# kmkolasinski/tfrecords-reader

Hardware: AMD Instinct MI355X
Metric: GiB/s + examples/s device-resident TFRecord->Feature decode, 1/2/4/8 GPU (higher is better)
Workload: dtype u8; 1 GPU; C4 directory (configs[4]) of 256 files, C1-shaped (int64 label + 12 B bytes_list id) records, 524288 +-50 % per file (default_rng(1000+f)), spec CRC-32C; this rank's LPT share (256 files) resident in HBM; records_per_gpu=134295581, framed_bytes_per_gpu=7906235019, parallelism=file-sharded x1 (LPT by bytes, no collective on the data path), batches_per_gpu=4, batch_bytes_max=1976558779, streams=2, tpl_groups_missed=0

## Files before the change

### include/tfrg.h

```cpp
#ifndef TFRG_H
#define TFRG_H
#include <stdint.h>
#include "tfrg_status.h"

#ifdef __cplusplus
extern "C" {
#endif

#define TFRG_ABI_VERSION 1

#define TFRG_E_ARG (-1)
#define TFRG_E_HIP (-2)
#define TFRG_E_NOMEM (-3)
#define TFRG_E_IO (-4)
#define TFRG_E_LIMIT (-5)

#define TFRG_FLAG_PAYLOAD_ONLY 1u
#define TFRG_FLAG_SPEC_VARINT 2u
#define TFRG_FLAG_NO_CRC 4u
#define TFRG_FLAG_STRICT_CRC 8u
#define TFRG_FLAG_MATERIALIZE_BYTES 16u

int tfrg_abi_version(void);
const char* tfrg_status_exception(int status);
// ... 104 lines not shown
  uint32_t n_miss_entries;
  uint32_t n_big;
  uint32_t scan_timeout;
  uint64_t kind_totals[4];
  uint64_t nbytes;
  uint64_t bytes_data_len;
  uint32_t tpl_groups_missed;
  uint32_t implicit_cols;
  uint64_t placed_slots;
  uint64_t implicit_off_slots;
} tfrg_info;

int tfrg_ctx_rel_off(const tfrg_ctx* ctx, uint32_t slot, int32_t* delta);

int tfrg_result_info(tfrg_ctx* ctx, tfrg_info* info);

typedef struct tfrg_columns {
  int32_t* status;
  int64_t* aux;
  uint8_t* verdict;
  uint16_t* order;
  uint32_t* row_splits;
  uint64_t* slot_base;
  int64_t* i64;
  uint32_t* f32;
  uint32_t* bytes_off;
  uint32_t* bytes_len;
  uint32_t* miss;
  uint8_t* bytes_data;
  uint64_t* bytes_offsets;
} tfrg_columns;

int tfrg_result_device(tfrg_ctx* ctx, tfrg_columns* cols);
int tfrg_result_fetch(tfrg_ctx* ctx, const tfrg_columns* host);

#define TFRG_DENSE_I64 0
#define TFRG_DENSE_I32 1
#define TFRG_DENSE_F32 2
#define TFRG_DENSE_U8 3
#define TFRG_DENSE_MAX_SPECS 64
#define TFRG_DENSE_MAX_WIDTH 4096
typedef struct tfrg_dense_spec {
  uint32_t slot;
  uint32_t dtype;
  uint32_t width;
  uint32_t reserved;
  uint64_t fill;
  void* out;
  int32_t* lengths;
} tfrg_dense_spec;
int tfrg_result_dense(tfrg_ctx* ctx, const tfrg_dense_spec* specs, uint32_t n_specs, uint32_t* d_stats,
                      void* consumer_stream);

#define TFRG_ROWS_I32 0
#define TFRG_ROWS_I64 1
int tfrg_result_dense_rows(tfrg_ctx* ctx, const tfrg_dense_spec* specs, uint32_t n_specs, const void* d_rows,
                           uint32_t rows_dtype, uint32_t m, int64_t row0, uint32_t* d_stats, uint32_t* d_skipped,
                           void* consumer_stream);

#define TFRG_RAGGED_MAX_SPECS 64
typedef struct tfrg_ragged_spec {
  uint32_t slot;
  uint32_t dtype;
  uint32_t max_len;
  uint32_t reserved;
  uint64_t cap;
// ... 58 lines not shown
```

### tfrecords-reader_amd/csrc/tfrg_capi.cpp

```cpp
#include <hip/hip_runtime.h>
#include <stdlib.h>
#include <string.h>

#include <algorithm>
#include <map>
#include <numeric>
#include <string>
#include <unordered_map>
#include <vector>

#include "../../include/tfrg.h"
#include "crc32c.h"
#include "tfrg_dense.h"
#include "tfrg_ragged.h"
#include "tfrg_select.h"
#include "tfrg_frame.h"
#include "tfrg_internal.h"
#include "tfrg_learn.h"

namespace tfrg {
void set_error(const std::string& s);

#define HIP_TRY(expr)                                                              \
  do {                                                                             \
    hipError_t e_ = (expr);                                                        \
    if (e_ != hipSuccess) {                                                        \
      set_error(std::string(#expr) + ": " + hipGetErrorString(e_));               \
      return TFRG_E_HIP;                                                           \
    }                                                                              \
  } while (0)

struct DBuf {
  void* p = nullptr;
  size_t cap = 0;
  hipError_t ensure(size_t bytes) {
    if (bytes <= cap && p) return hipSuccess;
    if (p) {
      hipError_t e = hipFree(p);
      if (e != hipSuccess) return e;
      p = nullptr;
      cap = 0;
    }
    size_t want = bytes < 256 ? 256 : bytes;
    want = (want + 4095) & ~(size_t)4095;
    hipError_t e = hipMalloc(&p, want);
    if (e == hipSuccess) cap = want;
    return e;
  }
  void release() {
    if (p) (void)hipFree(p);
    p = nullptr;
// ... 70 lines not shown
  uint32_t tpl_frames = 0;
  bool tpl_on = true;
  std::vector<uint8_t> slot_kind_h;
  DBuf spec;
  std::vector<uint32_t> spec_h;
  bool have_spec = false;
  bool spec_on = true;
  bool profiling = false;
  bool have_events = false;
  hipEvent_t ev[kNumStages + 1] = {};
  uint64_t hint_i64 = 0, hint_f32 = 0, hint_b = 0;
  bool hinted = false;
  bool no_hints = false;
  uint64_t hint_reruns = 0;
  bool optimistic_on = true;
  bool walk_beside = true;
  uint32_t walk_blocks = 0;
  bool no_quiet = false;
  bool opt_pending = false;
  bool ord_const = false;
  bool len_const = false;
  std::vector<uint32_t> const_len;
  bool implicit_off_on = true;
  uint64_t off_rel = 0;
  std::vector<int32_t> rel_off;
  uint64_t last_off_mask = 0;
  std::vector<int32_t> last_rel_off;
  bool off_complete = false;
  uint32_t last_implicit = 0;
  bool last_aux_zero = false;
  uint32_t* info_pin = nullptr;
  bool cols_complete = false;
  bool mat_pending = false;
  struct LastCall {
    const uint8_t* d_bytes;
    uint64_t nbytes;
    uint64_t cap_in;
    uint64_t bound;
    uint32_t n, flags;
    hipStream_t st;
  } last{};
  Offsets last_off{};
  uint32_t index_chunk = kIndexChunkDefault;
  DBuf fr_tab, fr_dev;
  uint32_t ragged_tile = kRaggedTileDefault;
  DBuf rg_tsum;
  uint32_t select_tile = kSelTileDefault;
  DBuf sel_buf;
  void* fr_pin = nullptr;
  size_t fr_pin_cap = 0;
  uint32_t poison[4] = {0xffffffffu, 0xffffffffu, 0xffffffffu, 0xffffffffu};
};

extern "C" {

int tfrg_ctx_create(int device, tfrg_ctx** out) {
  *out = nullptr;
  int ndev = 0;
  HIP_TRY(hipGetDeviceCount(&ndev));
  if (device < 0 || device >= ndev) {
    set_error("bad device index");
    return TFRG_E_ARG;
  }
  HIP_TRY(hipSetDevice(device));
  tfrg_ctx* c = new tfrg_ctx();
  c->device = device;
  if (const char* e = getenv("TFRG_TEMPLATES")) c->tpl_on = atoi(e) != 0;
  if (const char* e = getenv("TFRG_SPEC")) c->spec_on = atoi(e) != 0;
  if (const char* e = getenv("TFRG_TPL_STAGE")) c->tpl_stage = atoi(e);
  if (const char* e = getenv("TFRG_TPL_GPW")) {
    const int v = atoi(e);
    if (v == 2 || v == 4 || v == 8) c->tpl_gpw = (uint32_t)v;
  }
  if (const char* e = getenv("TFRG_OPTIMISTIC")) c->optimistic_on = atoi(e) != 0;
  if (const char* e = getenv("TFRG_IMPLICIT_OFF")) c->implicit_off_on = atoi(e) != 0;
  if (const char* e = getenv("TFRG_WALK_BESIDE")) c->walk_beside = atoi(e) != 0;
  if (const char* e = getenv("TFRG_WALK_BLOCKS")) c->walk_blocks = (uint32_t)atoi(e);
  if (const char* e = getenv("TFRG_DENSE_NT")) c->dense_nt = atoi(e) != 0;
  if (const char* e = getenv("TFRG_DEBUG_POISON_LOC")) {
    char* q = const_cast<char*>(e);
    for (int i = 0; i < 4 && *q; ++i) {
      c->poison[i] = (uint32_t)strtoul(q, &q, 10);
      while (*q == ',' || *q == ' ') ++q;
    }
  }
  hipDeviceProp_t prop;
  if (hipGetDeviceProperties(&prop, device) == hipSuccess) {
    c->num_cus = prop.multiProcessorCount;
    if (prop.maxSharedMemoryPerMultiProcessor) c->cu_lds = (uint32_t)prop.maxSharedMemoryPerMultiProcessor;
  }
  if (hipStreamCreateWithFlags(&c->own_stream, hipStreamNonBlocking) != hipSuccess) {
    delete c;
    set_error("hipStreamCreate failed");
    return TFRG_E_HIP;
  }
  if (hipHostMalloc(reinterpret_cast<void**>(&c->info_pin), (kInfoCount + 8) * 4) != hipSuccess) {
    (void)hipStreamDestroy(c->own_stream);
    delete c;
    set_error("hipHostMalloc failed");
    return TFRG_E_NOMEM;
  }
  std::vector<uint32_t> tab(kCrcTabWords), cst(128);
  CrcTables T;
  crc_make_tables(&T);
  memcpy(tab.data(), T.t, 4096);
  uint32_t M[4][256];
  crc_make_mul_tables(gf_xpow8(1024), M);
  memcpy(tab.data() + 1024, M, 4096);
// ... 421 lines not shown
  uint32_t* const info = c->info.as<uint32_t>() + c->info_slot * kInfoCount;
  DevBytes d;
  d.in = d_bytes;
  d.in_readable = (nbytes + 15) & ~15ull;
  d.b_off = c->b_off.as<uint32_t>();
  d.b_len = c->b_len.as<uint32_t>();
  d.kind_totals = c->kind_totals.as<uint64_t>();
  d.offsets = c->boff64.as<uint64_t>();
  d.offsets_cap = cap_b;
  d.data = c->bdata.as<uint8_t>();
  d.data_cap = cap_in + 16;
  d.lb = c->blb.as<uint64_t>();
  d.ticket = info + kInfoBytesTicket;
  d.big_count = info + kInfoBytesBig;
  d.big_list = c->bbig.as<uint32_t>();
  d.overflow = info + kInfoOverflow;
  return launch_materialize(d, c->num_cus, st);
}

static int decode_device_any(tfrg_ctx* c, const uint8_t* d_bytes, uint64_t nbytes, const Offsets& off, uint32_t n,
                             uint32_t flags, void* stream) {
  if (!c) return TFRG_E_ARG;
  if (nbytes >= (1ull << 32)) {
    set_error("batch larger than 4 GiB: split it");
    return TFRG_E_LIMIT;
  }
  if (c->n_keys == 0) {
    uint64_t z = 0;
    int st = tfrg_set_schema(c, 0, nullptr, &z, nullptr, 0, nullptr, nullptr);
    if (st) return st;
  }
  HIP_TRY(hipSetDevice(c->device));
  c->have_result = false;
  hipStream_t st = stream ? (hipStream_t)stream : c->own_stream;
  if (flags & TFRG_FLAG_STRICT_CRC) flags &= ~TFRG_FLAG_NO_CRC;
  if (c->last_stream && c->last_stream != st) {
    if (!c->order_ev) HIP_TRY(hipEventCreateWithFlags(&c->order_ev, hipEventDisableTiming));
    HIP_TRY(hipEventRecord(c->order_ev, c->last_stream));
    HIP_TRY(hipStreamWaitEvent(st, c->order_ev, 0));
  }
  const uint32_t S = c->n_slots;
  const uint64_t nn = n ? n : 1;
  const uint64_t ngroups = (nn + 63) / 64;
  const uint32_t n_tiles = (n + kTileRecs - 1) / kTileRecs;
  const uint32_t tile_stride = (n_tiles + 3u) & ~3u;
  const uint32_t n_chunks = (n_tiles + (1u << kSpineChunkShift) - 1u) >> kSpineChunkShift;
  const uint64_t tsum_words = (uint64_t)S * tile_stride + 2ull * S * n_chunks + S;
  const uint64_t cap_in = c->cap_hint > nbytes ? c->cap_hint : nbytes;
  c->cap_hint = 0;
  uint64_t cap_i64 = cap_in + 16, cap_f32 = cap_in / 4 + 16, cap_b = cap_in / 2 + 16;
  c->hinted = false;
  auto hint = [&](uint64_t h, uint64_t& cap) {
    if (h && h + 16 < cap) {
      cap = h + 16;
      c->hinted = true;
    }
  };
  if (!c->no_hints) {
    hint(c->hint_i64, cap_i64);
    hint(c->hint_f32, cap_f32);
    hint(c->hint_b, cap_b);
  }
  bool grow = c->status.cap < nn * 4 || c->aux.cap < nn * 8 || c->verdict.cap < nn ||
              c->order.cap < S * nn * 2 || c->count.cap < S * nn * 4 || c->loc.cap < S * nn * 8 ||
              c->rs.cap < S * (nn + 1) * 4 || c->i64.cap < cap_i64 * 8 || c->f32.cap < cap_f32 * 4 ||
              c->b_off.cap < cap_b * 4 || c->b_len.cap < cap_b * 4 || c->big_list.cap < nn * 4 ||
              c->slow_list.cap < nn * 4 || c->tsum.cap < tsum_words * 4 + 16 || c->crc_rec.cap < nn * 4 ||
              c->crc_base.cap < nn * 8 || c->crc_part.cap < nn * 8 || c->lmask.cap < ngroups * 8 ||
              c->rlist.cap < ngroups * 4;
  if (grow && c->last_stream) HIP_TRY(hipStreamSynchronize(c->last_stream));
  const size_t tsum_cap0 = c->tsum.cap;
  if (c->status.ensure(nn * 4) || c->aux.ensure(nn * 8) || c->verdict.ensure(nn) || c->order.ensure(S * nn * 2) ||
      c->count.ensure(S * nn * 4) || c->loc.ensure(S * nn * 8) || c->rs.ensure(S * (nn + 1) * 4) ||
      c->slot_base.ensure((S + 1) * 8) || c->totals.ensure((S + 1) * 4) || c->kind_totals.ensure(32) ||
      c->i64.ensure(cap_i64 * 8) || c->f32.ensure(cap_f32 * 4) || c->b_off.ensure(cap_b * 4) ||
      c->b_len.ensure(cap_b * 4) || c->big_list.ensure(nn * 4) || c->slow_list.ensure(nn * 4) ||
      c->miss.ensure(kMissCap * 16ull) || c->info.ensure(2 * kInfoCount * 4) ||
      c->tsum.ensure(tsum_words * 4 + 16) || c->crc_rec.ensure(nn * 4) || c->crc_base.ensure(nn * 8) ||
      c->crc_part.ensure(nn * 8) || c->lmask.ensure(ngroups * 8) || c->rlist.ensure(ngroups * 4)) {
    set_error("device allocation failed");
    return TFRG_E_NOMEM;
  }
  const uint32_t islot = c->info_slot ^ 1u;
  uint32_t* const info_cur = c->info.as<uint32_t>() + islot * kInfoCount;
  if (!c->info_clean) HIP_TRY(hipMemsetAsync(info_cur, 0, kInfoCount * 4, st));
  c->info_clean = false;
  c->info_slot = islot;
  if (c->tsum.cap != tsum_cap0 || c->tsum_dirty) {
    HIP_TRY(hipMemsetAsync(c->tsum.p, 0, c->tsum.cap, st));
    HIP_TRY(hipMemsetAsync(c->status.p, 0, c->status.cap, st));
    c->tsum_dirty = false;
  }
  if (S && n == 0) HIP_TRY(hipMemsetAsync(c->rs.p, 0, S * 4, st));
  const bool mat = (flags & TFRG_FLAG_MATERIALIZE_BYTES) != 0;
  const uint64_t lb_words = materialize_lb_words(cap_b);
  if (mat) {
    const bool g2 = c->bdata.cap < cap_in + 16 || c->boff64.cap < (cap_b + 1) * 8 || c->blb.cap < lb_words * 8 ||
                    c->bbig.cap < cap_b * 4;
    if (g2 && c->last_stream) HIP_TRY(hipStreamSynchronize(c->last_stream));
    if (c->bdata.ensure(cap_in + 16) || c->boff64.ensure((cap_b + 1) * 8) || c->blb.ensure(lb_words * 8) ||
        c->bbig.ensure(cap_b * 4)) {
      set_error("device allocation failed (materialized bytes)");
      return TFRG_E_NOMEM;
    }
    HIP_TRY(hipMemsetAsync(c->blb.p, 0, lb_words * 8, st));
    if (!n) HIP_TRY(hipMemsetAsync(c->boff64.p, 0, 8, st));
  }
  if (!S || !n) HIP_TRY(hipMemsetAsync(c->kind_totals.p, 0, 32, st));

  DevBatch b;
  b.bytes = d_bytes;
  b.nbytes = nbytes;
  b.start = off.s64;
  b.end = off.e64;
  b.start32 = off.s32;
  b.end32 = off.e32;
  b.first = off.first;
  b.omode = off.mode;
  b.n = n;
  b.flags = flags;
  DevOut o;
// ... 91 lines not shown
    }
    hipError_t e = launch_decode(b, schema_view(c), o, cfg, c->crc_tab.as<uint32_t>(), c->consts.as<uint32_t>(), st, ev);
    if (e == hipSuccess && mat && S && !cfg.ran_optimistic) {
      e = launch_materialize_last(c, d_bytes, nbytes, cap_in, cap_b, st);
    } else if (e == hipSuccess && mat && !S) {
      e = hipMemsetAsync(c->boff64.p, 0, 8, st);
    }
    if (ev && e == hipSuccess) e = hipEventRecord(ev[kNumStages], st);
    if (e != hipSuccess) {
      c->tsum_dirty = true;
      set_error(std::string("kernel launch: ") + hipGetErrorString(e));
      return TFRG_E_HIP;
    }
  }
  c->info_clean = n != 0;
  c->n = n;
  c->nbytes = nbytes;
  c->cap_i64 = cap_i64;
  c->cap_f32 = cap_f32;
  c->cap_b = cap_b;
  c->last_stream = st;
  c->materialized = mat;
  c->have_result = true;
  c->rs_complete = false;
  c->opt_pending = n != 0 && cfg.ran_optimistic;
  if (n != 0 && cfg.ran_quiet_big) c->tsum_dirty = true;
  c->mat_pending = c->opt_pending && mat && S;
  c->last_implicit = n != 0 ? cfg.implicit : 0u;
  c->last_off_mask = n != 0 ? cfg.implicit_off : 0ull;
  if (c->last_off_mask) c->last_rel_off = c->rel_off;
  c->off_complete = false;
  c->last_aux_zero = n != 0 && cfg.ran_optimistic && !cfg.ran_quiet_big && !(cfg.implicit & TFRG_IMPLICIT_STATUS);
  c->cols_complete = false;
  return 0;
}

int tfrg_decode_host(tfrg_ctx* c, const uint8_t* h_bytes, uint64_t nbytes, const uint64_t* h_start,
                     const uint64_t* h_end, uint32_t n, uint32_t flags, void* stream) {
  if (!c) return TFRG_E_ARG;
  HIP_TRY(hipSetDevice(c->device));
  hipStream_t st = stream ? (hipStream_t)stream : c->own_stream;
  const uint64_t pad = ((nbytes + 15) & ~15ull) + 16;
  if (c->last_stream) HIP_TRY(hipStreamSynchronize(c->last_stream));
  if (c->in_bytes.ensure(pad) || c->in_start.ensure((uint64_t)(n ? n : 1) * 8) ||
      c->in_end.ensure((uint64_t)(n ? n : 1) * 8)) {
    set_error("staging allocation failed");
    return TFRG_E_NOMEM;
  }
  if (nbytes) HIP_TRY(hipMemcpyAsync(c->in_bytes.p, h_bytes, nbytes, hipMemcpyHostToDevice, st));
  HIP_TRY(hipMemsetAsync(c->in_bytes.as<uint8_t>() + nbytes, 0, pad - nbytes, st));
  if (n) {
    HIP_TRY(hipMemcpyAsync(c->in_start.p, h_start, (size_t)n * 8, hipMemcpyHostToDevice, st));
    HIP_TRY(hipMemcpyAsync(c->in_end.p, h_end, (size_t)n * 8, hipMemcpyHostToDevice, st));
  }
  uint64_t total = 0, widest = 0;
  for (uint32_t i = 0; i < n; ++i) {
    const uint64_t a = h_start[i], b = h_end[i] < nbytes ? h_end[i] : nbytes;
    if (b > a) total += b - a;
    if (h_end[i] > a && h_end[i] - a > widest) widest = h_end[i] - a;
  }
  if (!c->tpl_learned && c->n_keys && c->tpl_on) {
    const int t = tfrg_learn_templates(c, h_bytes, nbytes, h_start, h_end, n, flags);
    if (t < 0) return t;
  }
  c->cap_hint = total;
  c->call_bound = widest ? widest : 1;
  return tfrg_decode_device(c, c->in_bytes.as<uint8_t>(), nbytes, c->in_start.as<uint64_t>(),
                            c->in_end.as<uint64_t>(), n, flags, st);
}

static int finish_decode(tfrg_ctx* c, uint32_t* h, uint64_t* kt) {
  bool widened = false;
  for (;;) {
    HIP_TRY(hipMemcpyAsync(c->info_pin, c->info.as<uint32_t>() + c->info_slot * kInfoCount, kInfoCount * 4,
                           hipMemcpyDeviceToHost, c->last_stream));
    HIP_TRY(hipMemcpyAsync(c->info_pin + kInfoCount, c->kind_totals.p, 32, hipMemcpyDeviceToHost, c->last_stream));
    HIP_TRY(hipStreamSynchronize(c->last_stream));
    memcpy(h, c->info_pin, kInfoCount * 4);
    memcpy(kt, c->info_pin + kInfoCount, 32);
    const bool full = c->opt_pending && h[kInfoResid] != 0;
    const bool widen = h[kInfoOverflow] && c->hinted && !widened;
    if (!full && !widen) {
      if (!c->mat_pending) break;
      c->mat_pending = false;
      const tfrg_ctx::LastCall& L = c->last;
      HIP_TRY(launch_materialize_last(c, L.d_bytes, L.nbytes, L.cap_in, c->cap_b, c->last_stream));
      continue;
    }
    const tfrg_ctx::LastCall L = c->last;
    c->no_quiet = true;
    c->no_hints = widen;
    c->cap_hint = L.cap_in;
    c->call_bound = L.bound;
    c->tsum_dirty = true;
    const int rc = decode_device_any(c, L.d_bytes, L.nbytes, c->last_off, L.n, L.flags, L.st);
    c->no_quiet = false;
    c->no_hints = false;
    if (rc) return rc;
    widened |= widen;
    ++c->hint_reruns;
  }
  c->opt_pending = false;
  c->hinted = false;
  return 0;
}

static int overflow_status(const uint32_t* h) {
  if (!h[kInfoOverflow]) return 0;
  set_error("value columns overflowed their capacity (overlapping ranges in a device batch): decode "
            "the ranges from host memory (tfrg_decode_host) or split the batch");
  return TFRG_E_LIMIT;
}

static int confirm_pending(tfrg_ctx* c) {
  if (!c->opt_pending && !c->hinted) return 0;
// ... 45 lines not shown
  std::vector<std::pair<uint64_t, uint32_t>> out;
  uint64_t base = 0;
  for (uint32_t k = 0; k < c->n_slots; ++k) {
    if ((c->slot_kind_h[k] & 3u) != TFRG_KIND_BYTES) continue;
    out.push_back({base, k < c->const_len.size() ? c->const_len[k] : 0u});
    base += c->n;
  }
  return out;
}

static std::vector<std::pair<uint64_t, uint32_t>> implicit_off_runs(const tfrg_ctx* c) {
  std::vector<std::pair<uint64_t, uint32_t>> out;
  uint64_t base = 0;
  for (uint32_t k = 0; k < c->n_slots; ++k) {
    if ((c->slot_kind_h[k] & 3u) != TFRG_KIND_BYTES) continue;
    if (k < 64u && ((c->last_off_mask >> k) & 1ull)) out.push_back({base, (uint32_t)c->last_rel_off[k]});
    base += c->n;
  }
  return out;
}

static int fill_implicit_off(tfrg_ctx* c) {
  if (!c->last_off_mask || c->off_complete || !c->n) return 0;
  HIP_TRY(hipSetDevice(c->device));
  for (const auto& [base, delta] : implicit_off_runs(c)) {
    if (base >= c->cap_b) continue;
    const uint32_t rows = (uint32_t)std::min<uint64_t>(c->n, c->cap_b - base);
    HIP_TRY(launch_fill_rel_off(c->b_off.as<uint32_t>() + base, c->last_off.e32, delta, rows, c->last_stream));
  }
  c->off_complete = true;
  return 0;
}

int tfrg_result_device(tfrg_ctx* c, tfrg_columns* d) {
  if (!c || !c->have_result) return TFRG_E_ARG;
  if (const int rc = confirm_pending(c)) return rc;
  if (!c->rs_complete && c->n_slots && c->n) {
    HIP_TRY(hipSetDevice(c->device));
    HIP_TRY(launch_fill_placed_rows(c->rs.as<uint32_t>(), c->info.as<uint32_t>() + c->info_slot * kInfoCount,
                                    c->n_slots, c->n, c->last_stream));
  }
  c->rs_complete = true;
  if ((c->last_implicit || c->last_aux_zero) && !c->cols_complete) {
    HIP_TRY(hipSetDevice(c->device));
    const size_t n = c->n;
    if (c->last_aux_zero) HIP_TRY(hipMemsetAsync(c->aux.p, 0, n * 8, c->last_stream));
    if (c->last_implicit & TFRG_IMPLICIT_STATUS) {
      HIP_TRY(hipMemsetAsync(c->status.p, 0, n * 4, c->last_stream));
      HIP_TRY(hipMemsetAsync(c->aux.p, 0, n * 8, c->last_stream));
      HIP_TRY(hipMemsetAsync(c->verdict.p, (int)(TFRG_V_LEN_MATCH | TFRG_V_LEN_CRC | TFRG_V_DATA_CRC), n, c->last_stream));
    }
    if (c->last_implicit & TFRG_IMPLICIT_ORDER)
      for (uint32_t k = 0; k < c->n_slots; ++k)
        HIP_TRY(hipMemsetD16Async(reinterpret_cast<hipDeviceptr_t>(c->order.as<uint16_t>() + (size_t)k * n),
                                  (unsigned short)(c->tpl_h[kLtSlot + 3 * k] >> 16), n, c->last_stream));
    if (c->last_implicit & TFRG_IMPLICIT_BYTES_LEN)
      for (const auto& [base, len] : implicit_len_runs(c))
        HIP_TRY(hipMemsetD32Async(reinterpret_cast<hipDeviceptr_t>(c->b_len.as<uint32_t>() + base), (int)len, n,
                                  c->last_stream));
  }
  c->cols_complete = true;
  if (const int rc = fill_implicit_off(c)) return rc;
  d->status = c->status.as<int32_t>();
  d->aux = c->aux.as<int64_t>();
  d->verdict = c->verdict.as<uint8_t>();
  d->order = c->order.as<uint16_t>();
  d->row_splits = c->rs.as<uint32_t>();
  d->slot_base = c->slot_base.as<uint64_t>();
  d->i64 = c->i64.as<int64_t>();
// ... 449 lines not shown
```

### tfrecords-reader_amd/csrc/tfrg_internal.h

```cpp
#pragma once
#include <stdint.h>
#include <hip/hip_runtime.h>
#include "tfrg_layout.h"

namespace tfrg {

struct DevSchema {
  uint32_t n_keys;
  uint32_t n_slots;
  uint32_t ht_mask;
  const uint32_t* ht;
  const uint32_t* key_hash;
  const uint32_t* key_off;
  const uint8_t* key_blob;
  const int32_t* key_slot;
  const uint8_t* slot_kind;
  const uint32_t* key_w;
  const uint32_t* krec;
  const uint32_t* tpl;
  const uint32_t* tpl_img;
  uint32_t tpl_img_words;
  uint32_t tpl_tab_words;
  uint32_t n_tpl;
  uint32_t tpl_w;
// ... 205 lines not shown
  bool ran_quiet_big;
  uint32_t tpl_cu_lds;
  bool tpl_stage_any;
  uint32_t tpl_gpw;
  bool walk_beside;
  uint32_t walk_blocks;
  uint32_t implicit;
  uint64_t off_rel;
  uint64_t implicit_off;
};

enum Stage : int { kStageTplLane = 0, kStageLaneCount, kStageBodyCount, kStageTailCount, kStageSpine,
                   kStageDownGather, kStageTailGather, kStageMaterialize, kNumStages };
extern const char* const kStageNames[kNumStages];

hipError_t launch_tpl_lane(const DevBatch& b, const DevOut& o, const LeanArgs& a, const uint32_t* img, uint32_t w,
                           int num_cus, hipStream_t st);
int lane_count_mode(const DevSchema& sc);
void launch_lane_count(const DevBatch& b, const DevSchema& sc, const DevOut& o, const uint32_t* d_tab,
                       const LaunchCfg& cfg, bool defer_big, int mode, int max_blocks, hipStream_t st);
void launch_body_count(const DevBatch& b, const DevOut& o, int num_cus, hipStream_t st);
bool tail_walk_fits(const DevSchema& sc);
void launch_tail_count(const DevBatch& b, const DevSchema& sc, const DevOut& o, const uint32_t* d_tab,
                       const uint32_t* d_consts, const LaunchCfg& cfg, bool finish, bool walk, uint32_t max_blocks,
                       hipStream_t st);
void launch_poison_loc(const DevOut& o, uint32_t n, uint32_t n_slots, const uint32_t recs[4], hipStream_t st);
void launch_spine(const DevOut& o, const DevSchema& sc, uint32_t n_tiles, uint32_t n, hipStream_t st);
void launch_down_gather(const DevBatch& b, const DevSchema& sc, const DevOut& o, const LaunchCfg& cfg,
                        uint32_t n_tiles, uint32_t resident, hipStream_t st);
void launch_tail_gather(const DevBatch& b, const DevSchema& sc, const DevOut& o, const LaunchCfg& cfg, int max_blocks,
                        hipStream_t st);
hipError_t launch_fill_placed_rows(uint32_t* rs, const uint32_t* info, uint32_t n_slots, uint32_t n, hipStream_t st);
hipError_t launch_fill_rel_off(uint32_t* off, const uint32_t* end32, uint32_t delta, uint32_t n, hipStream_t st);
hipError_t launch_stream_read(const void* d, uint64_t nbytes, uint32_t* sink, hipStream_t st, int variant);
struct FrTab;
hipError_t launch_frame_index(const FrTab& T, int num_cus, hipStream_t st);
hipError_t launch_decode(const DevBatch& b, const DevSchema& sc, const DevOut& o, LaunchCfg& cfg,
                         const uint32_t* d_crc_tables, const uint32_t* d_wave_consts, hipStream_t stream,
                         hipEvent_t* ev);

}
```

### tfrecords-reader_amd/csrc/tfrg_scan.hip

```cpp
#include <algorithm>
#include "tfrg_dev.h"

namespace tfrg {

constexpr int kSpineBlock = 256;
constexpr int kSpineItems = 16;
static_assert(kSpineBlock * kSpineItems == (1 << kSpineChunkShift), "one chunk per spine workgroup");

__device__ __forceinline__ uint32_t spine_look_back(const uint64_t* lb, uint32_t chunk, uint32_t lane) {
  uint32_t excl = 0;
  for (int64_t base = (int64_t)chunk - 1; base >= 0;) {
    const int64_t j = base - (int64_t)lane;
    const uint64_t w = j >= 0 ? __hip_atomic_load(&lb[j], __ATOMIC_RELAXED, __HIP_MEMORY_SCOPE_AGENT)
                              : (2ull << 32);
    const uint32_t flag = (uint32_t)(w >> 32);
    const uint64_t inc = __ballot(flag == 2u), unset = __ballot(flag == 0u);
    const uint32_t stop = inc ? (uint32_t)__builtin_ctzll(inc) : 64u;
    const uint64_t range = stop >= 63u ? ~0ull : (2ull << stop) - 1ull;
    if (unset & range) {
      __builtin_amdgcn_s_sleep(1);
      continue;
    }
    uint32_t v = lane <= stop ? (uint32_t)w : 0u;
#pragma unroll
    for (int m = 32; m >= 1; m >>= 1) v += (uint32_t)__shfl_xor((int)v, m, 64);
    excl += v;
    if (stop < 64u) break;
    base -= 64;
  }
  return excl;
}

__device__ __forceinline__ bool spec_failed(const uint32_t* spec, const DevOut& o, uint32_t k) {
  const uint32_t sw = spec ? spec[k] : 0u;
// ... 287 lines not shown
  hipLaunchKernelGGL(fn, dim3(ng < resident ? ng : resident), dim3(kLaneBlock), 0, st, b, sc, o, cfg.lane_max, n_tiles);
}

__global__ __launch_bounds__(256) void k_fill_placed_rows(uint32_t* __restrict__ rs, const uint32_t* __restrict__ info,
                                                          uint32_t n_slots, uint32_t n) {
  const uint64_t placed = ((uint64_t)info[kInfoPlacedHi] << 32) | info[kInfoPlacedLo];
  const uint32_t k = blockIdx.y;
  if (k >= 64u || k >= n_slots || !((placed >> k) & 1ull)) return;
  uint32_t* row = rs + (size_t)k * (n + 1u);
  for (uint32_t i = blockIdx.x * 256u + threadIdx.x; i <= n; i += gridDim.x * 256u) row[i] = i;
}

hipError_t launch_fill_placed_rows(uint32_t* rs, const uint32_t* info, uint32_t n_slots, uint32_t n, hipStream_t st) {
  const uint32_t slots = n_slots < 64u ? n_slots : 64u;
  if (!slots) return hipSuccess;
  const uint32_t blocks = (n + 1u + 255u) / 256u;
  hipLaunchKernelGGL(k_fill_placed_rows, dim3(blocks < 1024u ? blocks : 1024u, slots), dim3(256), 0, st, rs, info,
                     n_slots, n);
  return hipGetLastError();
}

__global__ __launch_bounds__(256) void k_fill_rel_off(uint32_t* __restrict__ off, const uint32_t* __restrict__ end32,
                                                      uint32_t delta, uint32_t n) {
  for (uint32_t i = blockIdx.x * 256u + threadIdx.x; i < n; i += gridDim.x * 256u) off[i] = end32[i] + delta;
}

hipError_t launch_fill_rel_off(uint32_t* off, const uint32_t* end32, uint32_t delta, uint32_t n, hipStream_t st) {
  if (!n) return hipSuccess;
  const uint32_t blocks = (n + 255u) / 256u;
  hipLaunchKernelGGL(k_fill_rel_off, dim3(blocks < 4096u ? blocks : 4096u), dim3(256), 0, st, off, end32, delta, n);
  return hipGetLastError();
}

}
```

### tfrecords-reader_amd/tfr_reader/_native.py

```python

from __future__ import annotations

import ctypes as C
import os
from pathlib import Path

_LIB: C.CDLL | None = None
_LIB_PATH = Path(os.environ.get("TFRG_LIB", Path(__file__).with_name("libtfrg.so")))

u8p = C.POINTER(C.c_uint8)
u16p = C.POINTER(C.c_uint16)
u32p = C.POINTER(C.c_uint32)
u64p = C.POINTER(C.c_uint64)
i32p = C.POINTER(C.c_int32)
i64p = C.POINTER(C.c_int64)


class TfrgInfo(C.Structure):
    _fields_ = [
        ("n_records", C.c_uint32),
        ("n_slots", C.c_uint32),
        ("n_errors", C.c_uint32),
        ("first_error", C.c_uint32),
        ("n_miss_records", C.c_uint32),
# ... 175 lines not shown
                                     C.c_int, C.c_uint32]),
    "tfrg_stream_wait": (C.c_int, [C.c_void_p, C.c_int, u64p, u64p, u64p, C.c_int, C.POINTER(C.c_double)]),
    "tfrg_stream_host_buffer": (C.c_void_p, [C.c_void_p, C.c_int]),
    "tfrg_stream_result": (C.c_int, [C.c_void_p, C.c_int, C.POINTER(TfrgInfo), C.POINTER(TfrgColumns)]),
    "tfrg_stream_host_ranges": (C.c_int, [C.c_void_p, C.c_int, C.POINTER(u64p), C.POINTER(u64p)]),
    "tfrg_ctx_set_profiling": (C.c_int, [C.c_void_p, C.c_int]),
    "tfrg_ctx_set_value_caps": (C.c_int, [C.c_void_p, C.c_uint64, C.c_uint64, C.c_uint64]),
    "tfrg_ctx_device_bytes": (C.c_int, [C.c_void_p, C.POINTER(C.c_uint64), C.POINTER(C.c_uint64)]),
    "tfrg_profile_last": (C.c_int, [C.c_void_p, C.POINTER(C.c_float), C.POINTER(C.c_char_p), C.c_int]),
    "tfrg_set_schema": (
        C.c_int,
        [C.c_void_p, C.c_uint32, C.c_void_p, u64p, u32p, C.c_uint32, u32p, u8p],
    ),
    "tfrg_decode_device": (
        C.c_int,
        [C.c_void_p, C.c_void_p, C.c_uint64, C.c_void_p, C.c_void_p, C.c_uint32, C.c_uint32, C.c_void_p],
    ),
    "tfrg_decode_device32": (
        C.c_int,
        [C.c_void_p, C.c_void_p, C.c_uint64, C.c_void_p, C.c_void_p, C.c_uint32, C.c_uint32, C.c_uint32,
         C.c_void_p],
    ),
    "tfrg_decode_host": (
        C.c_int,
        [C.c_void_p, C.c_void_p, C.c_uint64, u64p, u64p, C.c_uint32, C.c_uint32, C.c_void_p],
    ),
    "tfrg_ctx_set_index_chunk": (C.c_int, [C.c_void_p, C.c_uint32]),
    "tfrg_index_device": (C.c_int, [C.c_void_p, C.c_void_p, C.c_uint64, u64p, C.c_uint32, C.c_void_p, C.c_void_p,
                                    C.c_void_p, C.c_uint64, u64p, C.c_void_p, C.POINTER(TfrgIndexInfo)]),
    "tfrg_stream_set_device_index": (C.c_int, [C.c_void_p, C.c_int]),
    "tfrg_result_info": (C.c_int, [C.c_void_p, C.POINTER(TfrgInfo)]),
    "tfrg_ctx_rel_off": (C.c_int, [C.c_void_p, C.c_uint32, i32p]),
    "tfrg_result_device": (C.c_int, [C.c_void_p, C.POINTER(TfrgColumns)]),
    "tfrg_result_fetch": (C.c_int, [C.c_void_p, C.POINTER(TfrgColumns)]),
    "tfrg_result_dense": (C.c_int, [C.c_void_p, C.POINTER(TfrgDenseSpec), C.c_uint32, C.c_void_p, C.c_void_p]),
    "tfrg_result_dense_rows": (C.c_int, [C.c_void_p, C.POINTER(TfrgDenseSpec), C.c_uint32, C.c_void_p, C.c_uint32,
                                         C.c_uint32, C.c_int64, C.c_void_p, C.c_void_p, C.c_void_p]),
    "tfrg_result_ragged_rows": (C.c_int, [C.c_void_p, C.POINTER(TfrgRaggedSpec), C.c_uint32, C.c_void_p, C.c_uint32,
                                          C.c_uint32, C.c_int64, C.c_void_p, C.c_void_p, C.c_void_p]),
    "tfrg_ctx_set_ragged_tile": (C.c_int, [C.c_void_p, C.c_uint32]),
    "tfrg_result_select_rows": (C.c_int, [C.c_void_p, C.POINTER(TfrgSelectTerm), C.c_uint32, C.c_void_p, C.c_uint32,
                                          C.c_uint32, C.c_int64, C.c_void_p, C.c_uint32, C.c_uint64, C.c_void_p,
                                          C.c_void_p, C.c_uint32, C.c_void_p]),
    "tfrg_ctx_set_select_tile": (C.c_int, [C.c_void_p, C.c_uint32]),
}

FLAG_PAYLOAD_ONLY = 1
FLAG_SPEC_VARINT = 2
FLAG_NO_CRC = 4
FLAG_STRICT_CRC = 8
FLAG_MATERIALIZE_BYTES = 16


class NativeError(RuntimeError):
    pass


def lib() -> C.CDLL:
    global _LIB
    if _LIB is None:
        if not _LIB_PATH.exists():
            raise ImportError(
                f"libtfrg.so not found at {_LIB_PATH}: build it with "
                "`make -C tfrecords-reader_amd/csrc` (or __graft_entry__.build())"
            )
        lib_ = C.CDLL(str(_LIB_PATH))
# ... 17 lines not shown
```

### tfrecords-reader_amd/tfr_reader/hip.py

```python

from __future__ import annotations

import contextlib
import ctypes as C
import gc
import threading
from collections.abc import Sequence

import numpy as np

from tfr_reader import _native as N
from tfr_reader import _status as S

try:
    from tfr_reader import _tfrg_py as _PY
except ImportError:
    _PY = None

KIND_NAMES = {1: "bytes_list", 2: "float_list", 3: "int64_list"}


_GC_LOCK = threading.Lock()
_GC_DEPTH = 0
_GC_RESTORE = False
# ... 170 lines not shown

    def _flags(self, payload_only: bool, crc: bool, strict_crc: bool = False, materialize_bytes: bool = False) -> int:
        f = 0
        if payload_only:
            f |= N.FLAG_PAYLOAD_ONLY
        if self.spec_varint:
            f |= N.FLAG_SPEC_VARINT
        if not crc:
            f |= N.FLAG_NO_CRC
        if strict_crc:
            f |= N.FLAG_STRICT_CRC
        if materialize_bytes:
            f |= N.FLAG_MATERIALIZE_BYTES
        return f

    def info(self) -> N.TfrgInfo:
        info = N.TfrgInfo()
        N.check(self._lib.tfrg_result_info(self._ctx, C.byref(info)), "tfrg_result_info")
        return info

    def set_value_caps(self, int64_values: int = 0, float_values: int = 0, bytes_values: int = 0) -> None:
        N.check(self._lib.tfrg_ctx_set_value_caps(self._ctx, int(int64_values), int(float_values), int(bytes_values)),
                "tfrg_ctx_set_value_caps")

    def device_bytes(self) -> tuple[int, int]:
        b, r = C.c_uint64(), C.c_uint64()
        N.check(self._lib.tfrg_ctx_device_bytes(self._ctx, C.byref(b), C.byref(r)), "tfrg_ctx_device_bytes")
        return int(b.value), int(r.value)

    def device_columns(self) -> N.TfrgColumns:
        cols = N.TfrgColumns()
        N.check(self._lib.tfrg_result_device(self._ctx, C.byref(cols)), "tfrg_result_device")
        return cols

    def _learn_misses(self, buf: np.ndarray, info: N.TfrgInfo) -> bool:
        m = min(info.n_miss_entries, 1 << 16)
        miss = np.zeros((max(m, 1), 4), np.uint32)
        cols = N.TfrgColumns()
        cols.miss = N.ptr(miss, N.u32p)
        N.check(self._lib.tfrg_result_fetch(self._ctx, C.byref(cols)), "tfrg_result_fetch")
        new = False
        seen = set()
        for _rec, kind, off, ln in miss[:m].tolist():
            k = (off, ln, kind)
            if k in seen:
                continue
            seen.add(k)
            new |= self.keys.intern(bytes(buf[off : off + ln]), kind)
        return new

    SEED_SAMPLE = 64

    def _seed_keys(self, buf: np.ndarray, st: np.ndarray, en: np.ndarray, flags: int) -> None:
        n = int(st.shape[0])
        if n == 0 or buf.size == 0:
            return
        if n > self.SEED_SAMPLE:
            pick = np.linspace(0, n - 1, self.SEED_SAMPLE).astype(np.int64)
            st, en = np.ascontiguousarray(st[pick]), np.ascontiguousarray(en[pick])
        cap = 256
        out = np.zeros((cap, 3), np.uint64)
        k = int(self._lib.tfrg_scan_keys(N.ptr(buf), buf.size, N.ptr(st, N.u64p), N.ptr(en, N.u64p), st.size,
                                         flags & N.FLAG_PAYLOAD_ONLY, N.ptr(out, N.u64p), cap))
        for off, ln, kind in out[:k].tolist():
            self.keys.intern(bytes(buf[off : off + ln]), kind)

# ... 721 lines not shown
```

Baseline: 4720 GiB/s.

## Materialize implicit lean-decode columns with one fused fill kernel and cache them

On the lean optimistic decode path, constant or derivable columns (status, aux, verdict, order, lengths, row splits, relative offsets) are now filled by a single multi-segment fill kernel when results are requested, replacing several separate fill launches. A ViewState remembers which buffer ranges already hold the correct constant pattern from an earlier batch, so later batches with matching buffers skip rewriting them. Cached state is dropped whenever a buffer grows or the decode writes the column. This trades bookkeeping complexity and a risk of stale columns for fewer launches and less redundant HBM writing.

```diff
diff --git a/include/tfrg.h b/include/tfrg.h
--- a/include/tfrg.h
+++ b/include/tfrg.h
@@ -160,6 +160,7 @@
 } tfrg_columns;
 
 int tfrg_result_device(tfrg_ctx* ctx, tfrg_columns* cols);
+int tfrg_ctx_view_stats(const tfrg_ctx* ctx, uint64_t out[2]);
 int tfrg_result_fetch(tfrg_ctx* ctx, const tfrg_columns* host);
 
 #define TFRG_DENSE_I64 0
diff --git a/tfrecords-reader_amd/csrc/tfrg_capi.cpp b/tfrecords-reader_amd/csrc/tfrg_capi.cpp
--- a/tfrecords-reader_amd/csrc/tfrg_capi.cpp
+++ b/tfrecords-reader_amd/csrc/tfrg_capi.cpp
@@ -17,6 +17,7 @@
 #include "tfrg_frame.h"
 #include "tfrg_internal.h"
 #include "tfrg_learn.h"
+#include "tfrg_view.h"
 
 namespace tfrg {
 void set_error(const std::string& s);
@@ -153,6 +154,11 @@
   uint32_t* info_pin = nullptr;
   bool cols_complete = false;
   bool mat_pending = false;
+  ViewState view;
+  bool view_keep = true;
+  bool last_lean_opt = false;
+  uint64_t last_placed = 0;
+  uint64_t view_launches = 0, view_bytes = 0;
   struct LastCall {
     const uint8_t* d_bytes;
     uint64_t nbytes;
@@ -195,6 +201,7 @@
   }
   if (const char* e = getenv("TFRG_OPTIMISTIC")) c->optimistic_on = atoi(e) != 0;
   if (const char* e = getenv("TFRG_IMPLICIT_OFF")) c->implicit_off_on = atoi(e) != 0;
+  if (const char* e = getenv("TFRG_VIEW_KEEP")) c->view_keep = atoi(e) != 0;
   if (const char* e = getenv("TFRG_WALK_BESIDE")) c->walk_beside = atoi(e) != 0;
   if (const char* e = getenv("TFRG_WALK_BLOCKS")) c->walk_blocks = (uint32_t)atoi(e);
   if (const char* e = getenv("TFRG_DENSE_NT")) c->dense_nt = atoi(e) != 0;
@@ -682,6 +689,9 @@
   }
   HIP_TRY(hipSetDevice(c->device));
   c->have_result = false;
+  const ViewState view_before = c->view;
+  c->view.invalidate(kViewAll);
+  c->last_lean_opt = false;
   hipStream_t st = stream ? (hipStream_t)stream : c->own_stream;
   if (flags & TFRG_FLAG_STRICT_CRC) flags &= ~TFRG_FLAG_NO_CRC;
   if (c->last_stream && c->last_stream != st) {
@@ -720,6 +730,8 @@
               c->rlist.cap < ngroups * 4;
   if (grow && c->last_stream) HIP_TRY(hipStreamSynchronize(c->last_stream));
   const size_t tsum_cap0 = c->tsum.cap;
+  const size_t view_cap0[6] = {c->status.cap, c->aux.cap, c->verdict.cap, c->order.cap, c->b_len.cap, c->rs.cap};
+  uint32_t view_drop = 0;
   if (c->status.ensure(nn * 4) || c->aux.ensure(nn * 8) || c->verdict.ensure(nn) || c->order.ensure(S * nn * 2) ||
       c->count.ensure(S * nn * 4) || c->loc.ensure(S * nn * 8) || c->rs.ensure(S * (nn + 1) * 4) ||
       c->slot_base.ensure((S + 1) * 8) || c->totals.ensure((S + 1) * 4) || c->kind_totals.ensure(32) ||
@@ -736,7 +748,13 @@
   if (!c->info_clean) HIP_TRY(hipMemsetAsync(info_cur, 0, kInfoCount * 4, st));
   c->info_clean = false;
   c->info_slot = islot;
+  {
+    const size_t cap1[6] = {c->status.cap, c->aux.cap, c->verdict.cap, c->order.cap, c->b_len.cap, c->rs.cap};
+    for (int k = 0; k < 6; ++k)
+      if (cap1[k] != view_cap0[k]) view_drop |= 1u << k;
+  }
   if (c->tsum.cap != tsum_cap0 || c->tsum_dirty) {
+    view_drop |= kViewStatus;
     HIP_TRY(hipMemsetAsync(c->tsum.p, 0, c->tsum.cap, st));
     HIP_TRY(hipMemsetAsync(c->status.p, 0, c->status.cap, st));
     c->tsum_dirty = false;
@@ -894,6 +912,11 @@
   c->off_complete = false;
   c->last_aux_zero = n != 0 && cfg.ran_optimistic && !cfg.ran_quiet_big && !(cfg.implicit & TFRG_IMPLICIT_STATUS);
   c->cols_complete = false;
+  c->last_lean_opt = n != 0 && cfg.ran_optimistic && !cfg.ran_quiet_big && !mat;
+  if (c->last_lean_opt && c->view_keep) {
+    c->view = view_before;
+    c->view.invalidate(view_drop | lean_decode_stores(c->view, cfg.implicit, n));
+  }
   return 0;
 }
 
@@ -943,6 +966,7 @@
     const bool full = c->opt_pending && h[kInfoResid] != 0;
     const bool widen = h[kInfoOverflow] && c->hinted && !widened;
     if (!full && !widen) {
+      c->last_placed = ((uint64_t)h[kInfoPlacedHi] << 32) | h[kInfoPlacedLo];
       if (!c->mat_pending) break;
       c->mat_pending = false;
       const tfrg_ctx::LastCall& L = c->last;
@@ -1054,9 +1078,75 @@
   return 0;
 }
 
+static_assert(kViewMaxSlots == kLeanMaxSlots, "tfrg_view.h mirrors tfrg_layout.h");
+static ViewWant view_want(const tfrg_ctx* c) {
+  auto addr = [](const DBuf& b) { return (uint64_t)reinterpret_cast<uintptr_t>(b.p); };
+  ViewWant w;
+  w.n = c->n;
+  w.S = c->n_slots;
+  w.aux = addr(c->aux);
+  w.has_status = (c->last_implicit & TFRG_IMPLICIT_STATUS) != 0;
+  w.status = addr(c->status);
+  w.verdict = addr(c->verdict);
+  w.verdict_v = (uint8_t)(TFRG_V_LEN_MATCH | TFRG_V_LEN_CRC | TFRG_V_DATA_CRC);
+  w.has_order = (c->last_implicit & TFRG_IMPLICIT_ORDER) != 0;
+  w.order = addr(c->order);
+  for (uint32_t k = 0; w.has_order && k < c->n_slots && k < kViewMaxSlots; ++k)
+    w.order_c[k] = (uint16_t)(c->tpl_h[kLtSlot + 3 * k] >> 16);
+  w.rows = addr(c->rs);
+  w.placed = c->last_placed;
+  w.cap_b = c->cap_b;
+  w.has_len = (c->last_implicit & TFRG_IMPLICIT_BYTES_LEN) != 0;
+  w.len = addr(c->b_len);
+  if (w.has_len)
+    for (const auto& [base, len] : implicit_len_runs(c)) {
+      if (w.n_len >= kViewMaxSlots) break;
+      w.len_base[w.n_len] = base;
+      w.len_v[w.n_len++] = len;
+    }
+  w.off = addr(c->b_off);
+  if (c->last_off_mask && !c->off_complete)
+    for (const auto& [base, delta] : implicit_off_runs(c)) {
+      if (w.n_off >= kViewMaxSlots) break;
+      w.off_base[w.n_off] = base;
+      w.off_delta[w.n_off++] = delta;
+    }
+  return w;
+}
+
+static int fill_lean_view(tfrg_ctx* c) {
+  const ViewWant w = view_want(c);
+  ViewState s = c->view_keep ? c->view : ViewState{};
+  const ViewPlan plan = plan_view(s, w);
+  if (plan.nseg) {
+    HIP_TRY(hipSetDevice(c->device));
+    c->view.invalidate(kViewAll);
+    HIP_TRY(launch_fill_view(plan, c->last_off.e32, c->num_cus, c->last_stream));
+    ++c->view_launches;
+    c->view_bytes += plan.bytes();
+  }
+  if (c->view_keep) {
+    s.fold(w);
+    c->view = s;
+  }
+  return 0;
+}
+
+int tfrg_ctx_view_stats(const tfrg_ctx* c, uint64_t out[2]) {
+  if (!c || !out) return TFRG_E_ARG;
+  out[0] = c->view_launches;
+  out[1] = c->view_bytes;
+  return 0;
+}
+
 int tfrg_result_device(tfrg_ctx* c, tfrg_columns* d) {
   if (!c || !c->have_result) return TFRG_E_ARG;
   if (const int rc = confirm_pending(c)) return rc;
+  if (c->last_lean_opt && c->n) {
+    if (!c->cols_complete)
+      if (const int rc = fill_lean_view(c)) return rc;
+    c->rs_complete = c->cols_complete = c->off_complete = true;
+  }
   if (!c->rs_complete && c->n_slots && c->n) {
     HIP_TRY(hipSetDevice(c->device));
     HIP_TRY(launch_fill_placed_rows(c->rs.as<uint32_t>(), c->info.as<uint32_t>() + c->info_slot * kInfoCount,
diff --git a/tfrecords-reader_amd/csrc/tfrg_internal.h b/tfrecords-reader_amd/csrc/tfrg_internal.h
--- a/tfrecords-reader_amd/csrc/tfrg_internal.h
+++ b/tfrecords-reader_amd/csrc/tfrg_internal.h
@@ -261,6 +261,8 @@
                         hipStream_t st);
 hipError_t launch_fill_placed_rows(uint32_t* rs, const uint32_t* info, uint32_t n_slots, uint32_t n, hipStream_t st);
 hipError_t launch_fill_rel_off(uint32_t* off, const uint32_t* end32, uint32_t delta, uint32_t n, hipStream_t st);
+struct ViewPlan;
+hipError_t launch_fill_view(const ViewPlan& plan, const uint32_t* end32, int num_cus, hipStream_t st);
 hipError_t launch_stream_read(const void* d, uint64_t nbytes, uint32_t* sink, hipStream_t st, int variant);
 struct FrTab;
 hipError_t launch_frame_index(const FrTab& T, int num_cus, hipStream_t st);
diff --git a/tfrecords-reader_amd/csrc/tfrg_scan.hip b/tfrecords-reader_amd/csrc/tfrg_scan.hip
--- a/tfrecords-reader_amd/csrc/tfrg_scan.hip
+++ b/tfrecords-reader_amd/csrc/tfrg_scan.hip
@@ -1,5 +1,6 @@
 #include <algorithm>
 #include "tfrg_dev.h"
+#include "tfrg_view.h"
 
 namespace tfrg {
 
@@ -353,4 +354,111 @@
   return hipGetLastError();
 }
 
-}
+constexpr uint32_t kFillBlock = 256;
+
+struct FillSeg {
+  uint64_t addr;
+  uint64_t bytes;
+  uint64_t pat;
+  uint32_t row0;
+  uint32_t esize;
+  uint32_t kind;
+  uint32_t tile_end;
+};
+struct FillArgs {
+  const uint32_t* end32;
+  uint32_t nseg, ntiles;
+  FillSeg seg[kViewMaxSegs];
+};
+static_assert(sizeof(FillArgs) <= 4096, "passed by value");
+
+template <class T>
+__device__ __forceinline__ void fill_store(uint64_t addr, T v) {
+  *reinterpret_cast<T*>(addr) = v;
+}
+
+__device__ __forceinline__ uint32_t fill_elem32(const FillSeg& g, const uint32_t* __restrict__ end32, uint32_t row) {
+  return g.kind == kViewIdent ? row : end32[row] + (uint32_t)g.pat;
+}
+
+__device__ __forceinline__ uint4 fill_chunk(const FillSeg& g, const uint32_t* __restrict__ end32, uint64_t c) {
+  if (g.kind == kViewConst)
+    return make_uint4((uint32_t)g.pat, (uint32_t)(g.pat >> 32), (uint32_t)g.pat, (uint32_t)(g.pat >> 32));
+  const uint32_t r = g.row0 + (uint32_t)((c - g.addr) >> 2);
+  const uint32_t* src = end32 + r;
+  if (g.kind == kViewEndRel && !(reinterpret_cast<uintptr_t>(src) & 15u)) {
+    const uint4 x = *reinterpret_cast<const uint4*>(src);
+    const uint32_t d = (uint32_t)g.pat;
+    return make_uint4(x.x + d, x.y + d, x.z + d, x.w + d);
+  }
+  return make_uint4(fill_elem32(g, end32, r), fill_elem32(g, end32, r + 1u), fill_elem32(g, end32, r + 2u),
+                    fill_elem32(g, end32, r + 3u));
+}
+
+__device__ __forceinline__ void fill_edge(const FillSeg& g, const uint32_t* __restrict__ end32, uint64_t b, uint64_t e) {
+  for (uint64_t p = b; p < e; p += g.esize) {
+    if (g.kind != kViewConst) {
+      fill_store<uint32_t>(p, fill_elem32(g, end32, g.row0 + (uint32_t)((p - g.addr) >> 2)));
+    } else if (g.esize == 1u) {
+      fill_store<uint8_t>(p, (uint8_t)g.pat);
+    } else if (g.esize == 2u) {
+      fill_store<uint16_t>(p, (uint16_t)g.pat);
+    } else if (g.esize == 4u) {
+      fill_store<uint32_t>(p, (uint32_t)g.pat);
+    } else {
+      fill_store<uint64_t>(p, g.pat);
+    }
+  }
+}
+
+__global__ __launch_bounds__(kFillBlock) void k_fill_view(const FillArgs A) {
+  uint32_t s = 0, tile0 = 0;
+  for (uint32_t t = blockIdx.x; t < A.ntiles; t += gridDim.x) {
+    while (s + 1u < A.nseg && t >= A.seg[s].tile_end) tile0 = A.seg[s++].tile_end;
+    const FillSeg& g = A.seg[s];
+    const uint64_t lo = g.addr, hi = g.addr + g.bytes;
+    const uint64_t c = (lo & ~15ull) + ((uint64_t)(t - tile0) * kFillBlock + threadIdx.x) * 16ull;
+    if (c >= hi) continue;
+    if (c >= lo && c + 16u <= hi) {
+      fill_store<uint4>(c, fill_chunk(g, A.end32, c));
+    } else {
+      fill_edge(g, A.end32, c < lo ? lo : c, c + 16u > hi ? hi : c + 16u);
+    }
+  }
+}
+
+hipError_t launch_fill_view(const ViewPlan& plan, const uint32_t* end32, int num_cus, hipStream_t st) {
+  FillArgs A{};
+  A.end32 = end32;
+  A.nseg = 0;
+  uint64_t tiles = 0;
+  for (uint32_t i = 0; i < plan.nseg && A.nseg < kViewMaxSegs; ++i) {
+    const ViewSeg& v = plan.seg[i];
+    const uint32_t es = v.esize;
+    if (!v.rows || (es != 1u && es != 2u && es != 4u && es != 8u) || (v.kind != kViewConst && es != 4u) ||
+        (v.kind == kViewEndRel && !end32))
+      return hipErrorInvalidValue;
+    FillSeg& g = A.seg[A.nseg++];
+    g.addr = v.base + (uint64_t)v.first * es;
+    g.bytes = (uint64_t)v.rows * es;
+    if (g.addr % es) return hipErrorInvalidValue;
+    uint64_t pat = v.value;
+    if (v.kind == kViewConst)
+      for (uint32_t w = es; w < 8u; w *= 2u) pat = (pat & ((1ull << (8u * w)) - 1ull)) * ((1ull << (8u * w)) + 1ull);
+    g.pat = pat;
+    g.row0 = v.first;
+    g.esize = es;
+    g.kind = v.kind;
+    const uint64_t chunks = ((g.addr + g.bytes + 15u) >> 4) - (g.addr >> 4);
+    tiles += (chunks + kFillBlock - 1u) / kFillBlock;
+    if (tiles > 0xffffffffull) return hipErrorInvalidValue;
+    g.tile_end = (uint32_t)tiles;
+  }
+  if (!A.nseg) return hipSuccess;
+  A.ntiles = (uint32_t)tiles;
+  const uint64_t cap = (uint64_t)(num_cus > 0 ? num_cus : 1) * 8u;
+  hipLaunchKernelGGL(k_fill_view, dim3((uint32_t)(tiles < cap ? tiles : cap)), dim3(kFillBlock), 0, st, A);
+  return hipGetLastError();
+}
+
+}
diff --git a/tfrecords-reader_amd/csrc/tfrg_view.h b/tfrecords-reader_amd/csrc/tfrg_view.h
--- /dev/null
+++ b/tfrecords-reader_amd/csrc/tfrg_view.h
@@ -0,0 +1,178 @@
+#pragma once
+#include <stdint.h>
+
+namespace tfrg {
+
+constexpr uint32_t kViewMaxSlots = 16;
+constexpr uint32_t kViewMaxSegs = 3 + 2 * kViewMaxSlots + 2 * kViewMaxSlots;
+
+enum ViewCol : uint32_t {
+  kViewStatus = 1u, kViewAux = 2u, kViewVerdict = 4u, kViewOrder = 8u, kViewLen = 16u, kViewRows = 32u,
+  kViewAll = 63u,
+  kViewOff = 64u
+};
+enum ViewKind : uint32_t { kViewConst = 0, kViewIdent = 1, kViewEndRel = 2 };
+
+struct ViewSeg {
+  uint64_t base;
+  uint64_t value;
+  uint32_t first, rows;
+  uint32_t esize;
+  uint32_t kind;
+  uint32_t col;
+  uint64_t bytes() const { return (uint64_t)rows * (esize + (kind == kViewEndRel ? 4u : 0u)); }
+};
+
+struct ViewPlan {
+  uint32_t nseg = 0;
+  ViewSeg seg[kViewMaxSegs];
+  uint64_t bytes() const {
+    uint64_t b = 0;
+    for (uint32_t i = 0; i < nseg; ++i) b += seg[i].bytes();
+    return b;
+  }
+  void add(uint64_t base, uint64_t value, uint32_t first, uint32_t rows, uint32_t esize, uint32_t kind, uint32_t col) {
+    if (!rows || nseg >= kViewMaxSegs) return;
+    seg[nseg++] = ViewSeg{base, value, first, rows, esize, kind, col};
+  }
+};
+
+struct ViewWant {
+  uint32_t n = 0, S = 0;
+  uint64_t aux = 0;
+  bool has_status = false;
+  uint64_t status = 0, verdict = 0;
+  uint8_t verdict_v = 0;
+  bool has_order = false;
+  uint64_t order = 0;
+  uint16_t order_c[kViewMaxSlots] = {};
+  uint64_t rows = 0;
+  uint64_t placed = 0;
+  uint64_t cap_b = 0;
+  bool has_len = false;
+  uint64_t len = 0;
+  uint32_t n_len = 0;
+  uint64_t len_base[kViewMaxSlots] = {};
+  uint32_t len_v[kViewMaxSlots] = {};
+  uint64_t off = 0;
+  uint32_t n_off = 0;
+  uint64_t off_base[kViewMaxSlots] = {};
+  uint32_t off_delta[kViewMaxSlots] = {};
+};
+
+inline uint32_t view_run_rows(const ViewWant& w, uint64_t base) {
+  if (base >= w.cap_b) return 0u;
+  return w.cap_b - base < w.n ? (uint32_t)(w.cap_b - base) : w.n;
+}
+
+struct ViewState {
+  struct Rec {
+    uint64_t p = 0, value = 0;
+    uint32_t rows = 0;
+  } status, aux, verdict;
+  struct {
+    uint64_t p = 0;
+    uint32_t n = 0, S = 0;
+    uint16_t c[kViewMaxSlots] = {};
+  } order;
+  struct {
+    uint64_t p = 0;
+    uint32_t n = 0, runs = 0;
+    uint64_t base[kViewMaxSlots] = {};
+    uint32_t rows[kViewMaxSlots] = {};
+    uint32_t v[kViewMaxSlots] = {};
+  } len;
+  struct {
+    uint64_t p = 0, placed = 0;
+    uint32_t n = 0, S = 0;
+  } rows;
+
+  void invalidate(uint32_t mask) {
+    if (mask & kViewStatus) status = Rec{};
+    if (mask & kViewAux) aux = Rec{};
+    if (mask & kViewVerdict) verdict = Rec{};
+    if (mask & kViewOrder) order.p = 0;
+    if (mask & kViewLen) len.p = 0;
+    if (mask & kViewRows) rows.p = 0;
+  }
+
+  bool order_holds(const ViewWant& w) const {
+    if (!order.p || order.p != w.order || order.n != w.n || order.S != w.S) return false;
+    for (uint32_t k = 0; k < w.S && k < kViewMaxSlots; ++k)
+      if (order.c[k] != w.order_c[k]) return false;
+    return true;
+  }
+  bool len_holds(const ViewWant& w) const {
+    if (!len.p || len.p != w.len || len.n != w.n || len.runs != w.n_len) return false;
+    for (uint32_t j = 0; j < w.n_len && j < kViewMaxSlots; ++j)
+      if (len.base[j] != w.len_base[j] || len.v[j] != w.len_v[j] || len.rows[j] != view_run_rows(w, w.len_base[j]))
+        return false;
+    return true;
+  }
+  bool rows_hold(const ViewWant& w) const {
+    return rows.p && rows.p == w.rows && rows.n == w.n && rows.S == w.S && rows.placed == w.placed;
+  }
+
+  void fold(const ViewWant& w) {
+    auto rec = [&](Rec& r, uint64_t p, uint64_t value) {
+      const bool keep = r.p && r.p == p && r.value == value;
+      r = Rec{p, value, keep && r.rows > w.n ? r.rows : w.n};
+    };
+    rec(aux, w.aux, 0);
+    if (w.has_status) {
+      rec(status, w.status, 0);
+      rec(verdict, w.verdict, w.verdict_v);
+    }
+    if (w.has_order) {
+      order.p = w.order;
+      order.n = w.n;
+      order.S = w.S;
+      for (uint32_t k = 0; k < kViewMaxSlots; ++k) order.c[k] = k < w.S ? w.order_c[k] : 0;
+    }
+    if (w.has_len) {
+      len.p = w.len;
+      len.n = w.n;
+      len.runs = w.n_len;
+      for (uint32_t j = 0; j < kViewMaxSlots; ++j) {
+        len.base[j] = j < w.n_len ? w.len_base[j] : 0;
+        len.v[j] = j < w.n_len ? w.len_v[j] : 0;
+        len.rows[j] = j < w.n_len ? view_run_rows(w, w.len_base[j]) : 0;
+      }
+    }
+    rows.p = w.rows;
+    rows.placed = w.placed;
+    rows.n = w.n;
+    rows.S = w.S;
+  }
+};
+
+inline uint32_t lean_decode_stores(const ViewState& s, uint32_t implicit, uint32_t n) {
+  return ((implicit & 1u) ? 0u : (uint32_t)(kViewStatus | kViewVerdict)) | ((implicit & 2u) ? 0u : (uint32_t)kViewOrder) |
+         ((implicit & 4u) ? 0u : (uint32_t)kViewLen) | (s.rows.p && s.rows.n == n ? 0u : (uint32_t)kViewRows);
+}
+
+inline ViewPlan plan_view(const ViewState& s, const ViewWant& w) {
+  ViewPlan p;
+  if (!w.n) return p;
+  auto rec = [&](const ViewState::Rec& r, uint64_t base, uint64_t value, uint32_t esize, uint32_t col) {
+    const uint32_t have = r.p && r.p == base && r.value == value ? r.rows : 0u;
+    if (have < w.n) p.add(base, value, have, w.n - have, esize, kViewConst, col);
+  };
+  if (w.has_status) rec(s.status, w.status, 0, 4, kViewStatus);
+  rec(s.aux, w.aux, 0, 8, kViewAux);
+  if (w.has_status) rec(s.verdict, w.verdict, w.verdict_v, 1, kViewVerdict);
+  const uint32_t S = w.S < kViewMaxSlots ? w.S : kViewMaxSlots;
+  if (w.has_order && !s.order_holds(w))
+    for (uint32_t k = 0; k < S; ++k) p.add(w.order + 2ull * k * w.n, w.order_c[k], 0, w.n, 2, kViewConst, kViewOrder);
+  if (!s.rows_hold(w))
+    for (uint32_t k = 0; k < S; ++k)
+      if ((w.placed >> k) & 1ull) p.add(w.rows + 4ull * k * (w.n + 1ull), 0, 0, w.n + 1u, 4, kViewIdent, kViewRows);
+  if (w.has_len && !s.len_holds(w))
+    for (uint32_t j = 0; j < w.n_len && j < kViewMaxSlots; ++j)
+      p.add(w.len + 4ull * w.len_base[j], w.len_v[j], 0, view_run_rows(w, w.len_base[j]), 4, kViewConst, kViewLen);
+  for (uint32_t j = 0; j < w.n_off && j < kViewMaxSlots; ++j)
+    p.add(w.off + 4ull * w.off_base[j], w.off_delta[j], 0, view_run_rows(w, w.off_base[j]), 4, kViewEndRel, kViewOff);
+  return p;
+}
+
+}
diff --git a/tfrecords-reader_amd/tfr_reader/_native.py b/tfrecords-reader_amd/tfr_reader/_native.py
--- a/tfrecords-reader_amd/tfr_reader/_native.py
+++ b/tfrecords-reader_amd/tfr_reader/_native.py
@@ -231,6 +231,7 @@
     "tfrg_result_info": (C.c_int, [C.c_void_p, C.POINTER(TfrgInfo)]),
     "tfrg_ctx_rel_off": (C.c_int, [C.c_void_p, C.c_uint32, i32p]),
     "tfrg_result_device": (C.c_int, [C.c_void_p, C.POINTER(TfrgColumns)]),
+    "tfrg_ctx_view_stats": (C.c_int, [C.c_void_p, u64p]),
     "tfrg_result_fetch": (C.c_int, [C.c_void_p, C.POINTER(TfrgColumns)]),
     "tfrg_result_dense": (C.c_int, [C.c_void_p, C.POINTER(TfrgDenseSpec), C.c_uint32, C.c_void_p, C.c_void_p]),
     "tfrg_result_dense_rows": (C.c_int, [C.c_void_p, C.POINTER(TfrgDenseSpec), C.c_uint32, C.c_void_p, C.c_uint32,
diff --git a/tfrecords-reader_amd/tfr_reader/hip.py b/tfrecords-reader_amd/tfr_reader/hip.py
--- a/tfrecords-reader_amd/tfr_reader/hip.py
+++ b/tfrecords-reader_amd/tfr_reader/hip.py
@@ -226,6 +226,11 @@
         cols = N.TfrgColumns()
         N.check(self._lib.tfrg_result_device(self._ctx, C.byref(cols)), "tfrg_result_device")
         return cols
+
+    def view_stats(self) -> tuple[int, int]:
+        out = (C.c_uint64 * 2)()
+        N.check(self._lib.tfrg_ctx_view_stats(self._ctx, out), "tfrg_ctx_view_stats")
+        return int(out[0]), int(out[1])
 
     def _learn_misses(self, buf: np.ndarray, info: N.TfrgInfo) -> bool:
         m = min(info.n_miss_entries, 1 << 16)
```

Measured after the change: 4560 GiB/s. 3.4% lower.
